# microsoft/fadtk

Measured on AMD Instinct MI355X. Metric: FAD scores/sec + cov-GEMM TFLOP/s (% MFMA peak), N=100k D=512, higher is better.
Workload: dtype f16 in, f16 MFMA with f32 accumulate over <= 8192-row runs, f64 across runs (moments); split-f16 MFMA iterations (f32 accumulate) + exact int8-MFMA products (int32 accumulate) + f64 correction (Frechet)

## Files before the change

fadtk_amd/csrc/frechet.hip:

```cpp
#include "frechet_internal.h"
#include "ns_mean.h"
#include "ns_fast.h"
#include "ns_fast_big.h"
#include "ns_fast_res.h"

#include <algorithm>
#include <atomic>
#include <cmath>
#include <type_traits>

namespace fad {

Pool& thread_pool(int device) {
    static thread_local PerThreadDevice<Pool> set;
    return set.get(device);
}
Workspace* free_slot(int device) {
    Pool& p = thread_pool(device);
    for (Workspace& w : p.slot)
        if (!w.busy) { w.pool = &p; return &w; }
    return nullptr;
}

SongKnobs SongKnobs::from_env() {
    SongKnobs k;
    auto off = [](const char* name) { const char* e = getenv(name); return e && e[0] == '0'; };
    if (const char* e = getenv("FAD_SONG_BIG")) k.big_min = atol(e);
    if (const char* e = getenv("FAD_SONG_RES")) k.res = (e[0] == '0') ? 0 : (e[0] == '1' ? 1 : 2);
    if (const char* e = getenv("FAD_SONG_FAST")) k.fast = (e[0] == '0') ? 0 : (e[0] == '2' ? 2 : 1);
    if (const char* e = getenv("FAD_FAST_TRACE")) k.trace = e[0] == '1';
    k.scaled = !off("FAD_SONG_SCALED");
    if (const char* e = getenv("FAD_SONG_L0_SCALE")) { const double v = atof(e); if (v > 0.0) k.l0_scale = v; }
    return k;
}


struct MixedResult {
    int status;
    int iters, decided_at, nonfinite, too_few0, too_few1;
    double tr_scaled, c, tr1, tr2, mean_term, res, est;
    int prepared;
    int pad;
};

__global__ __launch_bounds__(256) void ns32_finish(const double* __restrict__ stats, int d, int nb,
                                                   const NsState* __restrict__ st, Ns32State* __restrict__ s32,
                                                   MixedResult* __restrict__ out, int max_low) {
    __shared__ double red[4];
    __shared__ double red3[12];
    const int tid = threadIdx.x;
    const bool live = s32->ok != 0;
    double mr = 0.0, mc = 0.0, corr = 0.0, r2 = 0.0, tr = 0.0;
    if (live) {
        const double* rowabs = stats;
        const double* colabs = stats + (int64_t)nb * d;
        const double* scal = stats + 2 * (int64_t)nb * d;
// ... 211 lines not shown
    g.B[0] = Rv; g.C[0] = Pv; g.C[1] = Ev;
    fast_split(d, nsf::SP_V2, g, st, B);
    g.B[0] = Pv; g.A[1] = Ev; g.C[0] = nsf::SplitMat{nullptr, nullptr}; g.C[1] = nsf::SplitMat{nullptr, nullptr};
    fast_split(d, nsf::SP_V3, g, st, B);
}
static void fast_split(int d, int mode, const nsf::SplitArgs& g, hipStream_t st, unsigned B) {
    const unsigned t = (unsigned)(d / 32);
    switch (d) {
        case 128: fast_launch_split<1>(mode, t, B, g, st); break;
        case 256: fast_launch_split<2>(mode, t, B, g, st); break;
        case 384: fast_launch_split<3>(mode, t, B, g, st); break;
        case 512: fast_launch_split<4>(mode, t, B, g, st); break;
        case 768: fast_launch_split<6>(mode, t, B, g, st); break;
        default: fast_launch_split<8>(mode, t, B, g, st); break;
    }
}
template <int NJ> static void fast_big_attrs() {
    (void)hipFuncSetAttribute(reinterpret_cast<const void*>(&nsf::nsf_big<nsf::SP_T, NJ>), hipFuncAttributeMaxDynamicSharedMemorySize, (int)nsf::kBigLds);
    (void)hipFuncSetAttribute(reinterpret_cast<const void*>(&nsf::nsf_big<nsf::SP_U, NJ>), hipFuncAttributeMaxDynamicSharedMemorySize, (int)nsf::kBigLds);
    (void)hipFuncSetAttribute(reinterpret_cast<const void*>(&nsf::nsf_big<nsf::SP_FIRST, NJ>), hipFuncAttributeMaxDynamicSharedMemorySize, (int)nsf::kBigLds);
}
template <int NJ> static void fast_big_launch(int d, int mode, const nsf::SplitArgs& g, hipStream_t st, unsigned B) {
    const int tt = nsf::big_tiles(d, NJ);
    const unsigned one = (unsigned)nsf::big_grid((int)B, tt), two = (unsigned)nsf::big_grid((int)B, 2 * tt);
    if (mode == nsf::SP_FIRST) hipLaunchKernelGGL((nsf::nsf_big<nsf::SP_FIRST, NJ>), dim3(one), dim3(256), nsf::kBigLds, st, g);
    else if (mode == nsf::SP_T) hipLaunchKernelGGL((nsf::nsf_big<nsf::SP_T, NJ>), dim3(one), dim3(256), nsf::kBigLds, st, g);
    else hipLaunchKernelGGL((nsf::nsf_big<nsf::SP_U, NJ>), dim3(two + B), dim3(256), nsf::kBigLds, st, g);
}
static int fast_big_t_slots(int d, unsigned B) { return nsf::big_tiles(d, nsf::big_nj(d, 1, (int)B)); }
static int fast_split_big(int d, int mode, nsf::SplitArgs g, hipStream_t st, unsigned B, int device) {
    static std::atomic<unsigned> ready{0};
    if (device >= 0 && device < 32 && !(ready.load(std::memory_order_acquire) & (1u << device))) {
        fast_big_attrs<1>(); fast_big_attrs<2>();
        FAD_HIP_TRY(hipGetLastError());
        ready.fetch_or(1u << device, std::memory_order_release);
    }
    g.nprob = (int)B;
    if (nsf::big_nj(d, mode == nsf::SP_U ? 2 : 1, (int)B) == 1) fast_big_launch<1>(d, mode, g, st, B);
    else fast_big_launch<2>(d, mode, g, st, B);
    return FAD_OK;
}
static int fast_i8_big(int d, int mode, const nsf::I8Args& g, hipStream_t st, unsigned B, int device) {
    static std::atomic<unsigned> ready{0};
    if (device >= 0 && device < 32 && !(ready.load(std::memory_order_acquire) & (1u << device))) {
        FAD_HIP_TRY(hipFuncSetAttribute(reinterpret_cast<const void*>(&nsf::nsf_i8_big<nsf::I8_A>), hipFuncAttributeMaxDynamicSharedMemorySize, (int)nsf::kI8BigLds));
        FAD_HIP_TRY(hipFuncSetAttribute(reinterpret_cast<const void*>(&nsf::nsf_i8_big<nsf::I8_G>), hipFuncAttributeMaxDynamicSharedMemorySize, (int)nsf::kI8BigLds));
        FAD_HIP_TRY(hipFuncSetAttribute(reinterpret_cast<const void*>(&nsf::nsf_i8_big<nsf::I8_G, true>), hipFuncAttributeMaxDynamicSharedMemorySize, (int)nsf::kI8BigLds));
        ready.fetch_or(1u << device, std::memory_order_release);
    }
    const unsigned grid = (unsigned)nsf::big_grid((int)B, (d / 128) * (d / 64));
    if (mode == nsf::I8_A) hipLaunchKernelGGL((nsf::nsf_i8_big<nsf::I8_A>), dim3(grid), dim3(512), nsf::kI8BigLds, st, g, (int)B);
    else if (g.Rv.a) hipLaunchKernelGGL((nsf::nsf_i8_big<nsf::I8_G, true>), dim3(grid), dim3(512), nsf::kI8BigLds, st, g, (int)B);
    else hipLaunchKernelGGL((nsf::nsf_i8_big<nsf::I8_G>), dim3(grid), dim3(512), nsf::kI8BigLds, st, g, (int)B);
    return FAD_OK;
}
template <int NS8> static void fast_launch_i8(int mode, unsigned t, unsigned B, const nsf::I8Args& g, hipStream_t st) {
    if (mode == nsf::I8_A) hipLaunchKernelGGL((nsf::nsf_i8<NS8, nsf::I8_A>), dim3(t, t, B), dim3(512), 0, st, g);
    else hipLaunchKernelGGL((nsf::nsf_i8<NS8, nsf::I8_G>), dim3(t, t, B), dim3(512), 0, st, g);
}
static void fast_i8(int d, int mode, const nsf::I8Args& g, hipStream_t st, unsigned B = 1) {
    const unsigned t = (unsigned)(d / 32);
    switch (d) {
        case 128: case 256: fast_launch_i8<1>(mode, t, B, g, st); break;
        case 384: case 512: fast_launch_i8<2>(mode, t, B, g, st); break;
        case 768: fast_launch_i8<3>(mode, t, B, g, st); break;
        default: fast_launch_i8<4>(mode, t, B, g, st); break;
    }
}

static nsf::SplitArgs fast_split_args(Workspace& ws, const MixedBufs& m, const FastBufs& f, int d) {
    nsf::SplitArgs g;
    memset(&g, 0, sizeof(g));
    g.d = d; g.gen = ws.job.gen; g.hA = f.hdr; g.hB = f.hdr + 1; g.st = m.dstate; g.s32 = m.s32;
    if (wide_enabled(ws.pool)) { g.scaled = 1; g.lp_wide = 1; g.l0_scale = kWideL0Scale; g.l0_min = kWideL0Min; }
    return g;
}
static int fast_verify_enqueue(Workspace& ws) {
    const int d = ws.job.d;
    MixedBufs m = mixed_bufs(ws, d);
    FastBufs f = fast_bufs(ws, d);
    f.host_words[13] = 0;
    fast_verify_launch(d, 1, fast_split_args(ws, m, f, d), f.Y, f.Z, f.Rv, f.Pv, f.Ev, m.s32, f.host_vstats, f.host_words, 0, ws.job.stream);
    FAD_HIP_TRY(hipGetLastError());
    FAD_HIP_TRY(hipEventRecord(ws.done_ev, ws.job.stream));
    return FAD_OK;
}
static int fast_enqueue(Workspace& ws, int upto) {
    const int d = ws.job.d;
    hipStream_t stream = ws.job.stream;
    MixedBufs m = mixed_bufs(ws, d);
    FastBufs f = fast_bufs(ws, d);
    if (!f.host_words) return set_error(FAD_ERR_ALLOC, "pinned result area of the fast Frechet chain is missing");
    const int nslots = (d / 32) * (d / 32);
    const int max_low = max_low_of(ws);
    for (int& k = ws.job.k; k < upto; ++k) {
        nsf::SplitArgs g = fast_split_args(ws, m, f, d);
        if (k == 0) {
            nsf::I8Args a;
            memset(&a, 0, sizeof(a));
            a.Adig = f.digC[0]; a.Bdig = f.digC[1]; a.d = d; a.gen = ws.job.gen; a.hA = f.hdr; a.hB = f.hdr + 1; a.stats = m.tilestats;
            a.A64 = m.A; a.P = f.P; a.st = m.dstate;
            fast_i8(d, nsf::I8_A, a, stream);
            g.A[0] = f.P; g.B[0] = f.P; g.C[0] = f.Y[1]; g.C[1] = f.Z[1]; g.Cdig[0] = f.digY[1]; g.Cdig_t[0] = f.digYt[1];
            g.A64 = m.A; g.statsA = m.tilestats;
            fast_split(d, nsf::SP_FIRST, g, stream, 1);
            continue;
// ... 360 lines not shown
    char* hpin = static_cast<char*>(ws.fast_pairs_pin);
    double* h_vals = reinterpret_cast<double*>(hpin);
    double* h_stats = h_vals + nsf::kHostVals;
    int* h_words = reinterpret_cast<int*>(h_stats + (size_t)(nsf::kTileStats + 2) * nb * nb);
    auto at = [&](size_t off) { return blk + off; };
    auto mat = [&](size_t off) { nsf::SplitMat m; m.a = reinterpret_cast<uint4*>(at(off)); m.at = reinterpret_cast<uint4*>(at(off + 4 * dd)); return m; };
    const int gen = ++ws.fast_gen;
    if (ws.fast_gen > (1 << 30)) ws.fast_gen = 1;
    ws.multi.gen = gen;
    if (ws.fast_pairs.p != before) {
        FAD_HIP_TRY(hipMemset2DAsync(at(L.hdrA), L.stride, 0, sizeof(nsf::MatHdr), (size_t)B, st));
        FAD_HIP_TRY(hipMemset2DAsync(at(L.hdrB), L.stride, 0, sizeof(nsf::MatHdr), (size_t)B, st));
    }
    nsf::MatHdr* hA = reinterpret_cast<nsf::MatHdr*>(at(L.hdrA));
    nsf::MatHdr* hB = reinterpret_cast<nsf::MatHdr*>(at(L.hdrB));
    NsState* st0 = reinterpret_cast<NsState*>(at(L.st));
    Ns32State* s32_0 = reinterpret_cast<Ns32State*>(at(L.s32));
    double* partials = reinterpret_cast<double*>(at(L.partials));
    double* stats = reinterpret_cast<double*>(at(L.stats));
    double* A64 = reinterpret_cast<double*>(at(L.A64));
    const nsf::SplitMat P = mat(L.P), Y[2] = {mat(L.Y[0]), mat(L.Y[1])}, Z[2] = {mat(L.Z[0]), mat(L.Z[1])}, T = mat(L.T);
    uint4* digY[2] = {reinterpret_cast<uint4*>(at(L.digY[0])), reinterpret_cast<uint4*>(at(L.digY[1]))};
    uint4* digYt[2] = {reinterpret_cast<uint4*>(at(L.digYt[0])), reinterpret_cast<uint4*>(at(L.digYt[1]))};

    static_assert(2 * kMaxMultiPairs <= nsf::kPrepMaxSets, "PrepArgs holds two sets per pair of a batch");
    nsf::PrepArgs pa;
    memset(&pa, 0, sizeof(pa));
    for (int b = 0; b < B; ++b) {
        pa.accs[2 * b] = moments_packed(h1[b]); pa.accs[2 * b + 1] = moments_packed(h2[b]);
        pa.runs[2 * b] = moments_runsum(h1[b]); pa.runs[2 * b + 1] = moments_runsum(h2[b]);
    }
    pa.acc[0] = pa.accs[0]; pa.acc[1] = pa.accs[1];
    pa.d = d; pa.ddof = ddof; pa.gen = gen; pa.mean_dtype = mean_dtype;
    pa.mus = reinterpret_cast<double*>(at(L.mus)); pa.covs = reinterpret_cast<double*>(at(L.covs));
    pa.dig[0] = reinterpret_cast<uint4*>(at(L.digA)); pa.dig[1] = reinterpret_cast<uint4*>(at(L.digB));
    pa.st = st0; pa.hdr[0] = hA; pa.hdr[1] = hB;
    pa.batch = 2; pa.pstride = (int64_t)L.stride; pa.no_covs = 1;
    pa.per = ((dd / 2048) % 4 == 0) ? 4 : 2;
    hipLaunchKernelGGL(nsf::nsf_prepare, dim3((unsigned)(dd / 2048 / pa.per + 1), (unsigned)(2 * B)), dim3(512), 0, st, pa);

    auto split_args = [&]() {
        nsf::SplitArgs g;
        memset(&g, 0, sizeof(g));
        g.d = d; g.gen = gen; g.hA = hA; g.hB = hB; g.pstride = (int64_t)L.stride; g.astride = (int64_t)L.stride;
        g.st = st0; g.s32 = s32_0;
        if (wide) { g.scaled = 1; g.lp_wide = 1; g.l0_scale = kWideL0Scale; g.l0_min = kWideL0Min; }
        return g;
    };
    {
        nsf::I8Args a;
        memset(&a, 0, sizeof(a));
        a.Adig = reinterpret_cast<uint4*>(at(L.digA)); a.Bdig = reinterpret_cast<uint4*>(at(L.digB)); a.d = d; a.gen = gen; a.hA = hA; a.hB = hB;
        a.pstride = (int64_t)L.stride; a.astride = (int64_t)L.stride; a.stats = stats; a.A64 = A64; a.P = P; a.st = st0;
        if (big) FAD_TRY(fast_i8_big(d, nsf::I8_A, a, st, (unsigned)B, device));
        else fast_i8(d, nsf::I8_A, a, st, (unsigned)B);
        nsf::SplitArgs g = split_args();
        g.A[0] = P; g.B[0] = P; g.C[0] = Y[1]; g.C[1] = Z[1]; g.A64 = A64; g.statsA = stats;
        if (big) FAD_TRY(fast_split_big(d, nsf::SP_FIRST, g, st, (unsigned)B, device));
        else { g.Cdig[0] = digY[1]; g.Cdig_t[0] = digYt[1]; fast_split(d, nsf::SP_FIRST, g, st, (unsigned)B); }
    }
    int want = ws.pool ? ws.pool->lp_iters : 5;
    if (want < 2) want = 2;
    if (want > max_low) want = max_low;
    for (int k = 1; k < want; ++k) {
        const int cur = k & 1;
        nsf::SplitArgs g = split_args();
        g.A[0] = Z[cur]; g.B[0] = Y[cur]; g.C[0] = T; g.alpha = -0.5f; g.beta_eye = 1.5f; g.gamma = 1.0f;
        g.partials = partials; g.skip = &s32_0->done; g.k = k;
        if (big) FAD_TRY(fast_split_big(d, nsf::SP_T, g, st, (unsigned)B, device));
        else fast_split(d, nsf::SP_T, g, st, (unsigned)B);
        g = split_args();
        g.A[0] = Y[cur]; g.B[0] = T; g.C[0] = Y[cur ^ 1]; g.A[1] = T; g.B[1] = Z[cur]; g.C[1] = Z[cur ^ 1];
        if (!big) { g.Cdig[0] = digY[cur ^ 1]; g.Cdig_t[0] = digYt[cur ^ 1]; }
        g.skip = &s32_0->upd_skip[k & 1];
        g.k = k; g.max_low = max_low; g.nslots = big ? fast_big_t_slots(d, (unsigned)B) : nb * nb; g.chk_partials = partials; g.thr_pred = pred_threshold(ws.pool, d);
        if (big) FAD_TRY(fast_split_big(d, nsf::SP_U, g, st, (unsigned)B, device));
        else fast_split(d, nsf::SP_U, g, st, (unsigned)B);
    }
    if (big) {
        nsf::DigArgs dg;
        memset(&dg, 0, sizeof(dg));
        dg.d = d; dg.gen = gen; dg.hA = hA; dg.hB = hB; dg.pstride = (int64_t)L.stride; dg.astride = (int64_t)L.stride; dg.s32 = s32_0;
        dg.Y[0] = Y[0]; dg.Y[1] = Y[1]; dg.dig[0] = digY[0]; dg.dig[1] = digY[1]; dg.dig_t[0] = digYt[0]; dg.dig_t[1] = digYt[1];
        hipLaunchKernelGGL(nsf::nsf_digitize, dim3((unsigned)((dd / 16 + 255) / 256), 2, (unsigned)B), dim3(256), 0, st, dg);
    }
    {
        nsf::I8Args a;
        memset(&a, 0, sizeof(a));
        a.Adig = digY[0]; a.Bdig = digYt[0]; a.Adig_alt = digY[1]; a.Bdig_alt = digYt[1]; a.sel = &s32_0->final_iter;
        a.d = d; a.gen = gen; a.hA = hA; a.hB = hB; a.pstride = (int64_t)L.stride; a.astride = (int64_t)L.stride; a.hstride = (int64_t)hs;
        a.skip = &s32_0->skip_corr; a.stats = h_stats; a.st = st0; a.A64in = A64;
        a.Y[0] = Y[0]; a.Y[1] = Y[1]; a.Z[0] = Z[0]; a.Z[1] = Z[1]; a.s32 = s32_0; a.host_words = h_words; a.host_vals = h_vals;
        if (wide) { a.Rv = mat(L.Rv); a.scaled = 1; }
        for (int b = 0; b < B; ++b) { int* w = reinterpret_cast<int*>(reinterpret_cast<char*>(h_words) + (size_t)b * hs); w[12] = 0; w[13] = 0; }
        if (big) FAD_TRY(fast_i8_big(d, nsf::I8_G, a, st, (unsigned)B, device));
        else fast_i8(d, nsf::I8_G, a, st, (unsigned)B);
    }
    FAD_HIP_TRY(hipGetLastError());
    if (!ws.done_ev) FAD_HIP_TRY(hipEventCreateWithFlags(&ws.done_ev, hipEventDisableTiming));
    if (wide && ws.pool && ws.pool->lp_verify) return pairs_verify_enqueue(ws, d, B, st);
    FAD_HIP_TRY(hipEventRecord(ws.done_ev, st));
    return FAD_OK;
}

static int mixed_begin(const NsProblem& pb, int device, hipStream_t stream, Workspace& ws) {
    const int d = pb.d;
    const int64_t dd = (int64_t)d * d;
    FAD_TRY(ws.mats.reserve((size_t)(6 * dd) * sizeof(double)));
    FAD_TRY(ws.mats32.reserve((size_t)(5 * dd) * sizeof(float)));
    const size_t hbytes = ws.job.fast ? fast_pinned_bytes(d) : sizeof(NsState) + sizeof(MixedResult);
    if (!ws.pinned || ws.pinned_cap < hbytes) {
        if (ws.pinned) (void)hipHostFree(ws.pinned);
        ws.pinned = nullptr; ws.pinned_cap = 0;
        FAD_HIP_TRY(hipHostMalloc(&ws.pinned, hbytes + 4096, hipHostMallocDefault));
        ws.pinned_cap = hbytes + 4096;
    }
    MixedBufs m = mixed_bufs(ws, d);
    m.hres->status = -1;
    ws.job.d = d; ws.job.device = device; ws.job.stream = stream; ws.job.k = 0;
    if (ws.job.fast) {
        ws.job.mu1 = pb.mu1; ws.job.mu2 = pb.mu2; ws.job.mean_dtype = pb.mean_dtype;
        int want = ws.pool ? ws.pool->lp_iters : 5;
        if (want < 2) want = 2;
        if (want > max_low_of(ws)) want = max_low_of(ws);
        if (ws.pool && ws.pool->lp_hopeless) want = 1;
        return fast_enqueue(ws, want);
    }
    NsProductExt ext;
    memset(&ext, 0, sizeof(ext));
    ext.stats = m.tilestats; ext.mu1 = pb.mu1; ext.mu2 = pb.mu2; ext.mean_dtype = pb.mean_dtype; ext.st = m.dstate;
    FAD_TRY(gemm_f64_product_stats_launch(d, pb.cov1, pb.cov2, m.A, &m.dstate->done, ext, stream));
    enqueue_ns_prepare(m.tilestats, d, (int)m.nb, pb.mu1, 0, pb.mu2, 0, pb.mean_dtype, m.dstate, 1, m.s32, 1, stream);
    int want = ws.pool ? ws.pool->lp_iters : 5;
    if (want < 2) want = 2;
    if (want > kMaxLow) want = kMaxLow;
    return mixed_enqueue(ws, want);
}

static int mixed_finish(Workspace& ws, MixedResult* res) {
    MixedBufs m = mixed_bufs(ws, ws.job.d);
    const int max_low = max_low_of(ws);
    bool asked = false;
    for (;;) {
        FAD_HIP_TRY(hipEventSynchronize(ws.done_ev));
        if (ws.job.fast) FAD_TRY(fast_decide(ws));
        if (m.hres->status == 5) {
            if (asked) { m.hres->status = 2; break; }
            asked = true;
// ... 383 lines not shown
```

fadtk_amd/csrc/ns_fast_big.h:

```cpp
#pragma once
#include "ns_fast.h"
#include "big_slots.h"

namespace fad {
namespace nsf {

#ifndef FAD_BIG_STAGES
#define FAD_BIG_STAGES 3
#endif
constexpr int kBigStages = FAD_BIG_STAGES;
constexpr int kBigStage = 1024;
constexpr size_t kBigLds = (size_t)kBigStages * kBigStage * 16 + 256;

template <int MODE, int NJ = 2>
__global__ __launch_bounds__(256, (FAD_BIG_STAGES <= 3) ? 3 : ((FAD_BIG_STAGES <= 4) ? 2 : 1)) void nsf_big(SplitArgs g) {
    static_assert(MODE == SP_T || MODE == SP_U || MODE == SP_FIRST, "SP_FIRST: iteration 0 (scale from nsf_i8<A>'s statistics, Y1, Z1)");
    extern __shared__ __attribute__((aligned(16))) uint4 ring[];
    double* red = reinterpret_cast<double*>(ring + kBigStages * kBigStage);
    const int d = g.d, tid = threadIdx.x, lane = tid & 63;
    constexpr int ZP = (MODE == SP_U) ? 2 : 1;
    const int t = d >> 7, tx_n = (NJ == 2) ? t : 2 * t, tt = t * tx_n;
    const int L = blockIdx.x;
    const int nprod = big_grid(g.nprob, tt * ZP);
    if constexpr (MODE == SP_U) {
// ... 176 lines not shown
                for (int reg = 0; reg < 16; ++reg) {
                    const int q = (reg & 3) + 8 * (reg >> 2);
                    const float y0 = (float)(A64[(int64_t)q * d] * inv_c);
                    const float y2 = (float)((double)(acc0[i][j][reg] + acc1[i][j][reg] * kLoInv) * (inv_cn * inv_cn));
                    fin[(q + 4 * kg) * 33 + r] = m1 * y0 - m3 * y2;
                    z1[reg] = ((by == bx && q + 4 * kg == r) ? m1 : 0.f) - m3 * y0;
                }
                __builtin_amdgcn_wave_barrier();
#pragma unroll
                for (int pass = 0; pass < 4; ++pass) store_tile_planes(fin, Cm, by, bx, d, pass * 64 + lane);
                __builtin_amdgcn_wave_barrier();
#pragma unroll
                for (int reg = 0; reg < 16; ++reg) fin[((reg & 3) + 8 * (reg >> 2) + 4 * kg) * 33 + r] = z1[reg];
                __builtin_amdgcn_wave_barrier();
                const SplitMat Zm1 = adv(g.C[1], po);
#pragma unroll
                for (int pass = 0; pass < 4; ++pass) store_tile_planes(fin, Zm1, by, bx, d, pass * 64 + lane);
                __builtin_amdgcn_wave_barrier();
                continue;
            }
            float ssf = 0.f;
#pragma unroll
            for (int reg = 0; reg < 16; ++reg) {
                const int q = (reg & 3) + 8 * (reg >> 2) + 4 * kg;
                const bool dg = (by == bx) && (q == r);
                const float v = alpha * (acc0[i][j][reg] + acc1[i][j][reg] * kLoInv) + (dg ? beta : 0.f);
                if constexpr (MODE == SP_T) { const float e = v - (dg ? gamma : 0.f); ssf = __builtin_fmaf(e, e, ssf); }
                fin[q * 33 + r] = v;
            }
            ss += (double)ssf;
            __builtin_amdgcn_wave_barrier();
#pragma unroll
            for (int pass = 0; pass < 4; ++pass) store_tile_planes(fin, Cm, by, bx, d, pass * 64 + lane);
            if (with_digits) {
#pragma unroll 2
                for (int pass = 0; pass < 8; ++pass) store_tile_digits(fin, dig, dig_t, by, bx, d, pass * 64 + lane);
            }
            __builtin_amdgcn_wave_barrier();
        }
    if constexpr (MODE == SP_T) {
        double s1[1] = {ss};
        wg8_sum<1, 4>(s1, red);
        if (tid == 0) adv(g.partials, po)[tile] = s1[0];
    }
}

constexpr int kI8BigStage = 36 * 64;
#ifndef FAD_I8_BIG_STAGES
#define FAD_I8_BIG_STAGES 2
#endif
constexpr int kI8BigStages = FAD_I8_BIG_STAGES;
constexpr size_t kI8BigLds = (size_t)kI8BigStages * kI8BigStage * 16 + 256;

template <int MODE, bool WITHR = false>
__global__ __launch_bounds__(512) void nsf_i8_big(I8Args g, int nprob) {
    extern __shared__ __attribute__((aligned(16))) uint4 ring[];
    double* red = reinterpret_cast<double*>(ring + kI8BigStages * kI8BigStage);
    constexpr int kUmin = (MODE == I8_A) ? kUminA : kUminG;
    constexpr int kGroups = 2 * (kDigits - 1) - kUmin + 1;
    const int d = g.d, tid = threadIdx.x, lane = tid & 63;
    const int tr_ = d >> 7, tc_ = d >> 6, tt = tr_ * tc_;
    const BigSlot slot = big_slot(blockIdx.x, nprob, tt);
    if (!slot.live) return;
    const int song = slot.song, tile = slot.item;
    const int TY = tile / tc_, TX = tile - TY * tc_;
    const int64_t po = (int64_t)song * g.pstride, ho = (int64_t)song * g.hstride;
    const MatHdr* hB = adv(g.hB, po);
    const MatHdr* hA = adv(g.hA, (int64_t)song * g.astride);
    NsState* const st_p = adv(g.st, po);
    const bool bad = hdr_bad(hA, hB, g.gen);
    const bool skipped = bad || (g.skip && *adv(g.skip, po) != 0);
    if constexpr (MODE == I8_G) {
        if (tile == 0 && tid == 0) {
            const NsState* st = st_p; const Ns32State* s = adv(g.s32, po);
            int* hw = adv(g.host_words, ho); double* hv = adv(g.host_vals, ho);
            hw[0] = bad ? 1 : 0; hw[1] = st->done; hw[2] = st->nonfinite; hw[3] = st->too_few[0]; hw[4] = st->too_few[1];
            hw[5] = s->ok; hw[6] = s->failed; hw[7] = s->final_iter; hw[8] = s->decided_at; hw[9] = s->strict; hw[10] = s->finished;
            hw[11] = skipped ? 1 : 0;
            hv[0] = st->c; hv[1] = st->tr1; hv[2] = st->tr2; hv[3] = st->mean_term;
#pragma unroll
            for (int q = 0; q < 16; ++q) hv[4 + q] = s->res[q];
            hw[14] = (g.scaled && st->mu[0] != 1.0) ? 1 : 0;
            hw[12] = g.gen;
        }
    }
    if (skipped) return;
    const int wave = __builtin_amdgcn_readfirstlane(tid >> 6);
    const int wr = wave >> 1, wc = wave & 1;
    const bool alt = (MODE == I8_G) && g.sel && (*adv(g.sel, po) & 1);
    const uint4* Ad = (MODE == I8_A) ? adv(g.Adig, (int64_t)song * g.astride) : adv(alt ? g.Adig_alt : g.Adig, po);
    const uint4* Bd = adv(alt ? g.Bdig_alt : g.Bdig, po);
#ifdef FAD_I8_ABL_G_NOLOOP
    const int nks = (MODE == I8_G) ? 0 : (d >> 5);
#else
    const int nks = d >> 5;
#endif

    const uint32_t voff = (uint32_t)lane * 16u;
    const uint32_t ring_lds = (uint32_t)(size_t)(__attribute__((address_space(3))) void*)ring;
    auto issue = [&](int ks) {
#pragma unroll
        for (int i = 0; i < 5; ++i) {
            const int q = wave + 8 * i;
            if (q < 36) {
                const bool bs = q >= 24;
                const int blk = bs ? (q - 24) / 6 : q / 6, p = bs ? (q - 24) % 6 : q % 6;
                const uint64_t sb = (uint64_t)((bs ? Bd : Ad) + dg_idx((bs ? 2 * TX : 4 * TY) + blk, ks, p, 0, d));
                const uint32_t lo = __builtin_amdgcn_readfirstlane((uint32_t)sb);
                const uint32_t hi = __builtin_amdgcn_readfirstlane((uint32_t)(sb >> 32));
                const uint64_t ub = ((uint64_t)hi << 32) | lo;
                const uint32_t m0v = __builtin_amdgcn_readfirstlane(ring_lds + (uint32_t)(((ks % kI8BigStages) * kI8BigStage + q * 64) * 16));
                asm volatile("s_mov_b32 m0, %2\n\ts_nop 0\n\tglobal_load_lds_dwordx4 %0, %1" ::"v"(voff), "s"(ub), "s"(m0v) : "memory", "m0");
            }
        }
    };
    i32x16 acc[kGroups];
#pragma unroll
    for (int u = 0; u < kGroups; ++u)
#pragma unroll
        for (int q = 0; q < 16; ++q) acc[u][q] = 0;
    static_assert(kI8BigStages >= 2 && kI8BigStages <= 4, "the counted waits below cover two younger stages at most");
    for (int ks = 0; ks < kI8BigStages - 1 && ks < nks; ++ks) issue(ks);
    const bool five = wave < 4;
    for (int ks = 0; ks < nks; ++ks) {
        const int ahead = (nks - 1 - ks < kI8BigStages - 2) ? (nks - 1 - ks) : (kI8BigStages - 2);
        if (ahead == 2) { if (five) asm volatile("s_waitcnt vmcnt(10)" ::: "memory"); else asm volatile("s_waitcnt vmcnt(8)" ::: "memory"); }
        else if (ahead == 1) { if (five) asm volatile("s_waitcnt vmcnt(5)" ::: "memory"); else asm volatile("s_waitcnt vmcnt(4)" ::: "memory"); }
        else asm volatile("s_waitcnt vmcnt(0)" ::: "memory");
        __builtin_amdgcn_s_barrier();
#ifndef FAD_I8_ABL_NODMA
        if (ks + kI8BigStages - 1 < nks) issue(ks + kI8BigStages - 1);
#endif
        const i32x4* st = reinterpret_cast<const i32x4*>(ring + (ks % kI8BigStages) * kI8BigStage) + lane;
        i32x4 a[kDigits], b[kDigits];
#pragma unroll
        for (int p = 0; p < kDigits; ++p) { a[p] = st[(wr * 6 + p) * 64]; b[p] = st[(24 + wc * 6 + p) * 64]; }
#ifdef FAD_I8_ABL_NOMMA
#pragma unroll
        for (int p = 0; p < kDigits; ++p) { acc[0][p] += a[p][0] ^ b[p][1]; acc[1][p] += a[p][2] ^ b[p][3]; }
#else
#pragma unroll
        for (int p = kDigits - 1; p >= 0; --p)
#pragma unroll
            for (int q = kDigits - 1; q >= 0; --q)
                if (p + q >= kUmin) acc[p + q - kUmin] = __builtin_amdgcn_mfma_i32_32x32x32_i8(a[p], b[q], acc[p + q - kUmin], 0, 0, 0);
#endif
    }
    __syncthreads();
    double gp[16];
#pragma unroll
    for (int q = 0; q < 16; ++q) gp[q] = 0.0;
#pragma unroll
    for (int u = 0; u < kGroups; ++u) {
        const double wgt = __builtin_ldexp(1.0, 7 * (u + kUmin) - 80);
#pragma unroll
        for (int q = 0; q < 16; ++q) gp[q] = __builtin_fma((double)acc[u][q], wgt, gp[q]);
    }
    float* fin = reinterpret_cast<float*>(ring) + wave * (32 * 33 + 32);
    const int kg = lane >> 5, n = lane & 31;
    const int by = 4 * TY + wr, bx = 2 * TX + wc, nb = d >> 5;
    const int row0 = 32 * by, col0 = 32 * bx;
    double* const stats = adv(g.stats, (MODE == I8_A) ? po : ho);
    double* scal = stats + (size_t)kTileStats * (by * nb + bx);
    double v3[3] = {0.0, 0.0, 0.0};
    if constexpr (MODE == I8_A) {
        const double inv = hdr_inv_s12(hA, hB);
        double* A64 = adv(g.A64, po) + (int64_t)(row0 + 4 * kg) * d + col0 + n;
#pragma unroll
        for (int reg = 0; reg < 16; ++reg) {
            const int q = (reg & 3) + 8 * (reg >> 2);
            A64[(int64_t)q * d] = gp[reg] * inv;
            fin[(q + 4 * kg) * 33 + n] = (float)gp[reg];
            v3[0] += gp[reg] * gp[reg];
            if (by == bx && q + 4 * kg == n) v3[1] += gp[reg];
        }
        __builtin_amdgcn_wave_barrier();
        const SplitMat Pm = adv(g.P, po);
#pragma unroll
        for (int pass = 0; pass < 4; ++pass) store_tile_planes(fin, Pm, by, bx, d, pass * 64 + lane);
    } else {
        const SplitMat Zm = adv(g.Z[alt ? 1 : 0], po);
        const SplitMat Ym = adv(g.Y[alt ? 1 : 0], po);
        const double inv_c = 1.0 / st_p->c;
        const double* A64 = adv(g.A64in, po) + (int64_t)(row0 + 4 * kg) * d + col0 + n;
        typedef _Float16 f16x4 __attribute__((ext_vector_type(4)));
        f16x4 zh[4], zl[4];
#pragma unroll
        for (int j = 0; j < 4; ++j) {
            int half;
            const size_t zi = fa_elem(col0 + n, row0 + 8 * j + 4 * kg, 0, d, half);
            zh[j] = *reinterpret_cast<const f16x4*>(reinterpret_cast<const _Float16*>(Zm.a + zi) + half);
            zl[j] = *reinterpret_cast<const f16x4*>(reinterpret_cast<const _Float16*>(Zm.a + zi + 64) + half);
        }
#pragma unroll
        for (int reg = 0; reg < 16; ++reg) {
            const int q = (reg & 3) + 8 * (reg >> 2), gr = row0 + q + 4 * kg, gc = col0 + n;
            const double R = A64[(int64_t)q * d] * inv_c - gp[reg];
            if constexpr (WITHR) gp[reg] = R;
            const double z = (double)used16(zh[reg >> 2][reg & 3], zl[reg >> 2][reg & 3]);
            v3[0] += z * R; v3[1] += R * R;
            if (by == bx && gr == gc) {
                int hy;
                const size_t yi = fa_elem(gr, gr, 0, d, hy);
                v3[2] += (double)used16(reinterpret_cast<const _Float16*>(Ym.a + yi)[hy], reinterpret_cast<const _Float16*>(Ym.a + yi + 64)[hy]);
            }
            fin[(q + 4 * kg) * 33 + n] = fabsf((float)z);
        }
        __builtin_amdgcn_wave_barrier();
    }
    double m = 0.0;
    if constexpr (MODE == I8_A) {
        if (lane < 32) { for (int c = 0; c < 32; ++c) m += fabsf(fin[lane * 33 + c]); }
        else { for (int q = 0; q < 32; ++q) m += fabsf(fin[q * 33 + lane - 32]); }
    } else {
        if (lane < 32) { for (int q = 0; q < 32; ++q) m += fin[q * 33 + lane]; }
        else { for (int c = 0; c < 32; ++c) m += fin[(lane - 32) * 33 + c]; }
    }
    double mrow = (lane < 32) ? m : 0.0, mcol = (lane >= 32) ? m : 0.0;
#pragma unroll
    for (int off = 32; off > 0; off >>= 1) {
        mrow = fmax(mrow, __shfl_xor(mrow, off)); mcol = fmax(mcol, __shfl_xor(mcol, off));
#pragma unroll
        for (int q = 0; q < 3; ++q) v3[q] += __shfl_xor(v3[q], off);
    }
    if (lane == 0) {
        if constexpr (MODE == I8_A) {
            scal[0] = v3[0]; scal[1] = v3[1]; scal[2] = mrow; scal[3] = mcol;
        } else {
            scal[0] = v3[0]; scal[1] = v3[1]; scal[2] = v3[2]; scal[3] = 0.0;
            double* zmax = stats + (size_t)kTileStats * nb * nb + 2 * (size_t)(by * nb + bx);
            zmax[0] = mrow; zmax[1] = mcol;
        }
    }
    if constexpr (MODE == I8_G && WITHR) {
        if (g.Rv.a) {
            __builtin_amdgcn_wave_barrier();
#pragma unroll
            for (int reg = 0; reg < 16; ++reg) fin[((reg & 3) + 8 * (reg >> 2) + 4 * kg) * 33 + n] = (float)(gp[reg] * (double)kVerScale);
            __builtin_amdgcn_wave_barrier();
            const SplitMat Rm = adv(g.Rv, po);
#pragma unroll
            for (int pass = 0; pass < 4; ++pass) store_tile_planes(fin, Rm, by, bx, d, pass * 64 + lane);
        }
    }
    (void)red;
}

}
}
```

Baseline: 12910.

## Add 64x64-tile int8 pair kernel with two-stage ring for big Frechet path

Adds a new int8 MFMA kernel for the big-matrix path. It uses 256 threads (4 waves covering a 64x64 output tile) instead of 512 threads on 128x64 tiles, with a two-stage LDS ring and launch bounds asking for 3 blocks per CU. The goal is more blocks in flight and a smaller LDS footprint, so more of the CUs stay busy at moderate d. In exchange each block reuses loaded digits less and the pipelining is shallower, since it waits on vmcnt(0) every k-step. The shared epilogue and per-problem setup are moved into helpers so both kernels can use them.

```diff
diff --git a/fadtk_amd/csrc/frechet.hip b/fadtk_amd/csrc/frechet.hip
--- a/fadtk_amd/csrc/frechet.hip
+++ b/fadtk_amd/csrc/frechet.hip
@@ -2,6 +2,7 @@
 #include "ns_mean.h"
 #include "ns_fast.h"
 #include "ns_fast_big.h"
+#include "ns_i8_pairs.h"
 #include "ns_fast_res.h"
 
 #include <algorithm>
@@ -319,6 +320,20 @@
     if (mode == nsf::I8_A) hipLaunchKernelGGL((nsf::nsf_i8_big<nsf::I8_A>), dim3(grid), dim3(512), nsf::kI8BigLds, st, g, (int)B);
     else if (g.Rv.a) hipLaunchKernelGGL((nsf::nsf_i8_big<nsf::I8_G, true>), dim3(grid), dim3(512), nsf::kI8BigLds, st, g, (int)B);
     else hipLaunchKernelGGL((nsf::nsf_i8_big<nsf::I8_G>), dim3(grid), dim3(512), nsf::kI8BigLds, st, g, (int)B);
+    return FAD_OK;
+}
+static int fast_i8_pairs(int d, int mode, const nsf::I8Args& g, hipStream_t st, unsigned B, int device) {
+    static std::atomic<unsigned> ready{0};
+    if (device >= 0 && device < 32 && !(ready.load(std::memory_order_acquire) & (1u << device))) {
+        FAD_HIP_TRY(hipFuncSetAttribute(reinterpret_cast<const void*>(&nsf::nsf_i8_pairs<nsf::I8_A>), hipFuncAttributeMaxDynamicSharedMemorySize, (int)nsf::kI8PairsLds));
+        FAD_HIP_TRY(hipFuncSetAttribute(reinterpret_cast<const void*>(&nsf::nsf_i8_pairs<nsf::I8_G>), hipFuncAttributeMaxDynamicSharedMemorySize, (int)nsf::kI8PairsLds));
+        FAD_HIP_TRY(hipFuncSetAttribute(reinterpret_cast<const void*>(&nsf::nsf_i8_pairs<nsf::I8_G, true>), hipFuncAttributeMaxDynamicSharedMemorySize, (int)nsf::kI8PairsLds));
+        ready.fetch_or(1u << device, std::memory_order_release);
+    }
+    const unsigned grid = (unsigned)nsf::big_grid((int)B, nsf::i8_pairs_tiles(d));
+    if (mode == nsf::I8_A) hipLaunchKernelGGL((nsf::nsf_i8_pairs<nsf::I8_A>), dim3(grid), dim3(256), nsf::kI8PairsLds, st, g, (int)B);
+    else if (g.Rv.a) hipLaunchKernelGGL((nsf::nsf_i8_pairs<nsf::I8_G, true>), dim3(grid), dim3(256), nsf::kI8PairsLds, st, g, (int)B);
+    else hipLaunchKernelGGL((nsf::nsf_i8_pairs<nsf::I8_G>), dim3(grid), dim3(256), nsf::kI8PairsLds, st, g, (int)B);
     return FAD_OK;
 }
 template <int NS8> static void fast_launch_i8(int mode, unsigned t, unsigned B, const nsf::I8Args& g, hipStream_t st) {
@@ -785,7 +800,7 @@
         memset(&a, 0, sizeof(a));
         a.Adig = reinterpret_cast<uint4*>(at(L.digA)); a.Bdig = reinterpret_cast<uint4*>(at(L.digB)); a.d = d; a.gen = gen; a.hA = hA; a.hB = hB;
         a.pstride = (int64_t)L.stride; a.astride = (int64_t)L.stride; a.stats = stats; a.A64 = A64; a.P = P; a.st = st0;
-        if (big) FAD_TRY(fast_i8_big(d, nsf::I8_A, a, st, (unsigned)B, device));
+        if (big) FAD_TRY(fast_i8_pairs(d, nsf::I8_A, a, st, (unsigned)B, device));
         else fast_i8(d, nsf::I8_A, a, st, (unsigned)B);
         nsf::SplitArgs g = split_args();
         g.A[0] = P; g.B[0] = P; g.C[0] = Y[1]; g.C[1] = Z[1]; g.A64 = A64; g.statsA = stats;
@@ -826,7 +841,7 @@
         a.Y[0] = Y[0]; a.Y[1] = Y[1]; a.Z[0] = Z[0]; a.Z[1] = Z[1]; a.s32 = s32_0; a.host_words = h_words; a.host_vals = h_vals;
         if (wide) { a.Rv = mat(L.Rv); a.scaled = 1; }
         for (int b = 0; b < B; ++b) { int* w = reinterpret_cast<int*>(reinterpret_cast<char*>(h_words) + (size_t)b * hs); w[12] = 0; w[13] = 0; }
-        if (big) FAD_TRY(fast_i8_big(d, nsf::I8_G, a, st, (unsigned)B, device));
+        if (big) FAD_TRY(fast_i8_pairs(d, nsf::I8_G, a, st, (unsigned)B, device));
         else fast_i8(d, nsf::I8_G, a, st, (unsigned)B);
     }
     FAD_HIP_TRY(hipGetLastError());
diff --git a/fadtk_amd/csrc/ns_fast_big.h b/fadtk_amd/csrc/ns_fast_big.h
--- a/fadtk_amd/csrc/ns_fast_big.h
+++ b/fadtk_amd/csrc/ns_fast_big.h
@@ -252,6 +252,151 @@
 constexpr int kI8BigStages = FAD_I8_BIG_STAGES;
 constexpr size_t kI8BigLds = (size_t)kI8BigStages * kI8BigStage * 16 + 256;
 
+struct I8Prob {
+    int64_t po, ho;
+    const MatHdr* hA; const MatHdr* hB;
+    NsState* st;
+    bool skipped, alt;
+};
+template <int MODE>
+__device__ __forceinline__ I8Prob i8_problem(const I8Args& g, int song, bool first) {
+    I8Prob pb;
+    const int64_t po = (int64_t)song * g.pstride, ho = (int64_t)song * g.hstride;
+    pb.po = po; pb.ho = ho;
+    pb.hB = adv(g.hB, po);
+    pb.hA = adv(g.hA, (int64_t)song * g.astride);
+    pb.st = adv(g.st, po);
+    const bool bad = hdr_bad(pb.hA, pb.hB, g.gen);
+    const bool skipped = bad || (g.skip && *adv(g.skip, po) != 0);
+    pb.skipped = skipped;
+    if constexpr (MODE == I8_G) {
+        if (first) {
+            const NsState* st = pb.st; const Ns32State* s = adv(g.s32, po);
+            int* hw = adv(g.host_words, ho); double* hv = adv(g.host_vals, ho);
+            hw[0] = bad ? 1 : 0; hw[1] = st->done; hw[2] = st->nonfinite; hw[3] = st->too_few[0]; hw[4] = st->too_few[1];
+            hw[5] = s->ok; hw[6] = s->failed; hw[7] = s->final_iter; hw[8] = s->decided_at; hw[9] = s->strict; hw[10] = s->finished;
+            hw[11] = skipped ? 1 : 0;
+            hv[0] = st->c; hv[1] = st->tr1; hv[2] = st->tr2; hv[3] = st->mean_term;
+#pragma unroll
+            for (int q = 0; q < 16; ++q) hv[4 + q] = s->res[q];
+            hw[14] = (g.scaled && st->mu[0] != 1.0) ? 1 : 0;
+            hw[12] = g.gen;
+        }
+    }
+    pb.alt = false;
+    if constexpr (MODE == I8_G) { if (!skipped) pb.alt = g.sel && (*adv(g.sel, po) & 1); }
+    return pb;
+}
+
+template <int MODE, bool WITHR, int NG>
+__device__ __forceinline__ void i8_block_epilogue(const I8Args& g, const I8Prob& pb, const i32x16 (&acc)[NG], uint4* ring, int by, int bx, int wave) {
+    constexpr int kUmin = (MODE == I8_A) ? kUminA : kUminG;
+    constexpr int kGroups = NG;
+    static_assert(NG == 2 * (kDigits - 1) - kUmin + 1, "one accumulator per digit-pair weight");
+    const int d = g.d, lane = threadIdx.x & 63;
+    const int64_t po = pb.po, ho = pb.ho;
+    const MatHdr* hA = pb.hA; const MatHdr* hB = pb.hB;
+    const NsState* st_p = pb.st;
+    const bool alt = pb.alt;
+    __syncthreads();
+    double gp[16];
+#pragma unroll
+    for (int q = 0; q < 16; ++q) gp[q] = 0.0;
+#pragma unroll
+    for (int u = 0; u < kGroups; ++u) {
+        const double wgt = __builtin_ldexp(1.0, 7 * (u + kUmin) - 80);
+#pragma unroll
+        for (int q = 0; q < 16; ++q) gp[q] = __builtin_fma((double)acc[u][q], wgt, gp[q]);
+    }
+    float* fin = reinterpret_cast<float*>(ring) + wave * (32 * 33 + 32);
+    const int kg = lane >> 5, n = lane & 31;
+    const int nb = d >> 5;
+    const int row0 = 32 * by, col0 = 32 * bx;
+    double* const stats = adv(g.stats, (MODE == I8_A) ? po : ho);
+    double* scal = stats + (size_t)kTileStats * (by * nb + bx);
+    double v3[3] = {0.0, 0.0, 0.0};
+    if constexpr (MODE == I8_A) {
+        const double inv = hdr_inv_s12(hA, hB);
+        double* A64 = adv(g.A64, po) + (int64_t)(row0 + 4 * kg) * d + col0 + n;
+#pragma unroll
+        for (int reg = 0; reg < 16; ++reg) {
+            const int q = (reg & 3) + 8 * (reg >> 2);
+            A64[(int64_t)q * d] = gp[reg] * inv;
+            fin[(q + 4 * kg) * 33 + n] = (float)gp[reg];
+            v3[0] += gp[reg] * gp[reg];
+            if (by == bx && q + 4 * kg == n) v3[1] += gp[reg];
+        }
+        __builtin_amdgcn_wave_barrier();
+        const SplitMat Pm = adv(g.P, po);
+#pragma unroll
+        for (int pass = 0; pass < 4; ++pass) store_tile_planes(fin, Pm, by, bx, d, pass * 64 + lane);
+    } else {
+        const SplitMat Zm = adv(g.Z[alt ? 1 : 0], po);
+        const SplitMat Ym = adv(g.Y[alt ? 1 : 0], po);
+        const double inv_c = 1.0 / st_p->c;
+        const double* A64 = adv(g.A64in, po) + (int64_t)(row0 + 4 * kg) * d + col0 + n;
+        typedef _Float16 f16x4 __attribute__((ext_vector_type(4)));
+        f16x4 zh[4], zl[4];
+#pragma unroll
+        for (int j = 0; j < 4; ++j) {
+            int half;
+            const size_t zi = fa_elem(col0 + n, row0 + 8 * j + 4 * kg, 0, d, half);
+            zh[j] = *reinterpret_cast<const f16x4*>(reinterpret_cast<const _Float16*>(Zm.a + zi) + half);
+            zl[j] = *reinterpret_cast<const f16x4*>(reinterpret_cast<const _Float16*>(Zm.a + zi + 64) + half);
+        }
+#pragma unroll
+        for (int reg = 0; reg < 16; ++reg) {
+            const int q = (reg & 3) + 8 * (reg >> 2), gr = row0 + q + 4 * kg, gc = col0 + n;
+            const double R = A64[(int64_t)q * d] * inv_c - gp[reg];
+            if constexpr (WITHR) gp[reg] = R;
+            const double z = (double)used16(zh[reg >> 2][reg & 3], zl[reg >> 2][reg & 3]);
+            v3[0] += z * R; v3[1] += R * R;
+            if (by == bx && gr == gc) {
+                int hy;
+                const size_t yi = fa_elem(gr, gr, 0, d, hy);
+                v3[2] += (double)used16(reinterpret_cast<const _Float16*>(Ym.a + yi)[hy], reinterpret_cast<const _Float16*>(Ym.a + yi + 64)[hy]);
+            }
+            fin[(q + 4 * kg) * 33 + n] = fabsf((float)z);
+        }
+        __builtin_amdgcn_wave_barrier();
+    }
+    double m = 0.0;
+    if constexpr (MODE == I8_A) {
+        if (lane < 32) { for (int c = 0; c < 32; ++c) m += fabsf(fin[lane * 33 + c]); }
+        else { for (int q = 0; q < 32; ++q) m += fabsf(fin[q * 33 + lane - 32]); }
+    } else {
+        if (lane < 32) { for (int q = 0; q < 32; ++q) m += fin[q * 33 + lane]; }
+        else { for (int c = 0; c < 32; ++c) m += fin[(lane - 32) * 33 + c]; }
+    }
+    double mrow = (lane < 32) ? m : 0.0, mcol = (lane >= 32) ? m : 0.0;
+#pragma unroll
+    for (int off = 32; off > 0; off >>= 1) {
+        mrow = fmax(mrow, __shfl_xor(mrow, off)); mcol = fmax(mcol, __shfl_xor(mcol, off));
+#pragma unroll
+        for (int q = 0; q < 3; ++q) v3[q] += __shfl_xor(v3[q], off);
+    }
+    if (lane == 0) {
+        if constexpr (MODE == I8_A) {
+            scal[0] = v3[0]; scal[1] = v3[1]; scal[2] = mrow; scal[3] = mcol;
+        } else {
+            scal[0] = v3[0]; scal[1] = v3[1]; scal[2] = v3[2]; scal[3] = 0.0;
+            double* zmax = stats + (size_t)kTileStats * nb * nb + 2 * (size_t)(by * nb + bx);
+            zmax[0] = mrow; zmax[1] = mcol;
+        }
+    }
+    if constexpr (MODE == I8_G && WITHR) {
+        if (g.Rv.a) {
+            __builtin_amdgcn_wave_barrier();
+#pragma unroll
+            for (int reg = 0; reg < 16; ++reg) fin[((reg & 3) + 8 * (reg >> 2) + 4 * kg) * 33 + n] = (float)(gp[reg] * (double)kVerScale);
+            __builtin_amdgcn_wave_barrier();
+            const SplitMat Rm = adv(g.Rv, po);
+#pragma unroll
+            for (int pass = 0; pass < 4; ++pass) store_tile_planes(fin, Rm, by, bx, d, pass * 64 + lane);
+        }
+    }
+}
+
 template <int MODE, bool WITHR = false>
 __global__ __launch_bounds__(512) void nsf_i8_big(I8Args g, int nprob) {
     extern __shared__ __attribute__((aligned(16))) uint4 ring[];
@@ -264,30 +409,12 @@
     if (!slot.live) return;
     const int song = slot.song, tile = slot.item;
     const int TY = tile / tc_, TX = tile - TY * tc_;
-    const int64_t po = (int64_t)song * g.pstride, ho = (int64_t)song * g.hstride;
-    const MatHdr* hB = adv(g.hB, po);
-    const MatHdr* hA = adv(g.hA, (int64_t)song * g.astride);
-    NsState* const st_p = adv(g.st, po);
-    const bool bad = hdr_bad(hA, hB, g.gen);
-    const bool skipped = bad || (g.skip && *adv(g.skip, po) != 0);
-    if constexpr (MODE == I8_G) {
-        if (tile == 0 && tid == 0) {
-            const NsState* st = st_p; const Ns32State* s = adv(g.s32, po);
-            int* hw = adv(g.host_words, ho); double* hv = adv(g.host_vals, ho);
-            hw[0] = bad ? 1 : 0; hw[1] = st->done; hw[2] = st->nonfinite; hw[3] = st->too_few[0]; hw[4] = st->too_few[1];
-            hw[5] = s->ok; hw[6] = s->failed; hw[7] = s->final_iter; hw[8] = s->decided_at; hw[9] = s->strict; hw[10] = s->finished;
-            hw[11] = skipped ? 1 : 0;
-            hv[0] = st->c; hv[1] = st->tr1; hv[2] = st->tr2; hv[3] = st->mean_term;
-#pragma unroll
-            for (int q = 0; q < 16; ++q) hv[4 + q] = s->res[q];
-            hw[14] = (g.scaled && st->mu[0] != 1.0) ? 1 : 0;
-            hw[12] = g.gen;
-        }
-    }
-    if (skipped) return;
+    const I8Prob pb = i8_problem<MODE>(g, song, tile == 0 && tid == 0);
+    if (pb.skipped) return;
+    const int64_t po = pb.po;
     const int wave = __builtin_amdgcn_readfirstlane(tid >> 6);
     const int wr = wave >> 1, wc = wave & 1;
-    const bool alt = (MODE == I8_G) && g.sel && (*adv(g.sel, po) & 1);
+    const bool alt = pb.alt;
     const uint4* Ad = (MODE == I8_A) ? adv(g.Adig, (int64_t)song * g.astride) : adv(alt ? g.Adig_alt : g.Adig, po);
     const uint4* Bd = adv(alt ? g.Bdig_alt : g.Bdig, po);
 #ifdef FAD_I8_ABL_G_NOLOOP
@@ -346,103 +473,7 @@
                 if (p + q >= kUmin) acc[p + q - kUmin] = __builtin_amdgcn_mfma_i32_32x32x32_i8(a[p], b[q], acc[p + q - kUmin], 0, 0, 0);
 #endif
     }
-    __syncthreads();
-    double gp[16];
-#pragma unroll
-    for (int q = 0; q < 16; ++q) gp[q] = 0.0;
-#pragma unroll
-    for (int u = 0; u < kGroups; ++u) {
-        const double wgt = __builtin_ldexp(1.0, 7 * (u + kUmin) - 80);
-#pragma unroll
-        for (int q = 0; q < 16; ++q) gp[q] = __builtin_fma((double)acc[u][q], wgt, gp[q]);
-    }
-    float* fin = reinterpret_cast<float*>(ring) + wave * (32 * 33 + 32);
-    const int kg = lane >> 5, n = lane & 31;
-    const int by = 4 * TY + wr, bx = 2 * TX + wc, nb = d >> 5;
-    const int row0 = 32 * by, col0 = 32 * bx;
-    double* const stats = adv(g.stats, (MODE == I8_A) ? po : ho);
-    double* scal = stats + (size_t)kTileStats * (by * nb + bx);
-    double v3[3] = {0.0, 0.0, 0.0};
-    if constexpr (MODE == I8_A) {
-        const double inv = hdr_inv_s12(hA, hB);
-        double* A64 = adv(g.A64, po) + (int64_t)(row0 + 4 * kg) * d + col0 + n;
-#pragma unroll
-        for (int reg = 0; reg < 16; ++reg) {
-            const int q = (reg & 3) + 8 * (reg >> 2);
-            A64[(int64_t)q * d] = gp[reg] * inv;
-            fin[(q + 4 * kg) * 33 + n] = (float)gp[reg];
-            v3[0] += gp[reg] * gp[reg];
-            if (by == bx && q + 4 * kg == n) v3[1] += gp[reg];
-        }
-        __builtin_amdgcn_wave_barrier();
-        const SplitMat Pm = adv(g.P, po);
-#pragma unroll
-        for (int pass = 0; pass < 4; ++pass) store_tile_planes(fin, Pm, by, bx, d, pass * 64 + lane);
-    } else {
-        const SplitMat Zm = adv(g.Z[alt ? 1 : 0], po);
-        const SplitMat Ym = adv(g.Y[alt ? 1 : 0], po);
-        const double inv_c = 1.0 / st_p->c;
-        const double* A64 = adv(g.A64in, po) + (int64_t)(row0 + 4 * kg) * d + col0 + n;
-        typedef _Float16 f16x4 __attribute__((ext_vector_type(4)));
-        f16x4 zh[4], zl[4];
-#pragma unroll
-        for (int j = 0; j < 4; ++j) {
-            int half;
-            const size_t zi = fa_elem(col0 + n, row0 + 8 * j + 4 * kg, 0, d, half);
-            zh[j] = *reinterpret_cast<const f16x4*>(reinterpret_cast<const _Float16*>(Zm.a + zi) + half);
-            zl[j] = *reinterpret_cast<const f16x4*>(reinterpret_cast<const _Float16*>(Zm.a + zi + 64) + half);
-        }
-#pragma unroll
-        for (int reg = 0; reg < 16; ++reg) {
-            const int q = (reg & 3) + 8 * (reg >> 2), gr = row0 + q + 4 * kg, gc = col0 + n;
-            const double R = A64[(int64_t)q * d] * inv_c - gp[reg];
-            if constexpr (WITHR) gp[reg] = R;
-            const double z = (double)used16(zh[reg >> 2][reg & 3], zl[reg >> 2][reg & 3]);
-            v3[0] += z * R; v3[1] += R * R;
-            if (by == bx && gr == gc) {
-                int hy;
-                const size_t yi = fa_elem(gr, gr, 0, d, hy);
-                v3[2] += (double)used16(reinterpret_cast<const _Float16*>(Ym.a + yi)[hy], reinterpret_cast<const _Float16*>(Ym.a + yi + 64)[hy]);
-            }
-            fin[(q + 4 * kg) * 33 + n] = fabsf((float)z);
-        }
-        __builtin_amdgcn_wave_barrier();
-    }
-    double m = 0.0;
-    if constexpr (MODE == I8_A) {
-        if (lane < 32) { for (int c = 0; c < 32; ++c) m += fabsf(fin[lane * 33 + c]); }
-        else { for (int q = 0; q < 32; ++q) m += fabsf(fin[q * 33 + lane - 32]); }
-    } else {
-        if (lane < 32) { for (int q = 0; q < 32; ++q) m += fin[q * 33 + lane]; }
-        else { for (int c = 0; c < 32; ++c) m += fin[(lane - 32) * 33 + c]; }
-    }
-    double mrow = (lane < 32) ? m : 0.0, mcol = (lane >= 32) ? m : 0.0;
-#pragma unroll
-    for (int off = 32; off > 0; off >>= 1) {
-        mrow = fmax(mrow, __shfl_xor(mrow, off)); mcol = fmax(mcol, __shfl_xor(mcol, off));
-#pragma unroll
-        for (int q = 0; q < 3; ++q) v3[q] += __shfl_xor(v3[q], off);
-    }
-    if (lane == 0) {
-        if constexpr (MODE == I8_A) {
-            scal[0] = v3[0]; scal[1] = v3[1]; scal[2] = mrow; scal[3] = mcol;
-        } else {
-            scal[0] = v3[0]; scal[1] = v3[1]; scal[2] = v3[2]; scal[3] = 0.0;
-            double* zmax = stats + (size_t)kTileStats * nb * nb + 2 * (size_t)(by * nb + bx);
-            zmax[0] = mrow; zmax[1] = mcol;
-        }
-    }
-    if constexpr (MODE == I8_G && WITHR) {
-        if (g.Rv.a) {
-            __builtin_amdgcn_wave_barrier();
-#pragma unroll
-            for (int reg = 0; reg < 16; ++reg) fin[((reg & 3) + 8 * (reg >> 2) + 4 * kg) * 33 + n] = (float)(gp[reg] * (double)kVerScale);
-            __builtin_amdgcn_wave_barrier();
-            const SplitMat Rm = adv(g.Rv, po);
-#pragma unroll
-            for (int pass = 0; pass < 4; ++pass) store_tile_planes(fin, Rm, by, bx, d, pass * 64 + lane);
-        }
-    }
+    i8_block_epilogue<MODE, WITHR>(g, pb, acc, ring, 4 * TY + wr, 2 * TX + wc, wave);
     (void)red;
 }
 
diff --git a/fadtk_amd/csrc/ns_i8_pairs.h b/fadtk_amd/csrc/ns_i8_pairs.h
--- /dev/null
+++ b/fadtk_amd/csrc/ns_i8_pairs.h
@@ -0,0 +1,72 @@
+#pragma once
+#include "ns_fast_big.h"
+
+namespace fad {
+namespace nsf {
+
+constexpr int kI8PairsStage = 24 * 64;
+constexpr int kI8PairsStages = 2;
+constexpr size_t kI8PairsLds = (size_t)kI8PairsStages * kI8PairsStage * 16 + 256;
+constexpr int i8_pairs_tiles(int d) { return (d >> 6) * (d >> 6); }
+static_assert(4 * (32 * 33 + 32) * sizeof(float) <= (size_t)kI8PairsStages * kI8PairsStage * 16, "the epilogue's four [32][33] areas live in the ring");
+
+template <int MODE, bool WITHR = false>
+__global__ __launch_bounds__(256, 3) void nsf_i8_pairs(I8Args g, int nprob) {
+    extern __shared__ __attribute__((aligned(16))) uint4 ring[];
+    constexpr int kUmin = (MODE == I8_A) ? kUminA : kUminG;
+    constexpr int kGroups = 2 * (kDigits - 1) - kUmin + 1;
+    const int d = g.d, tid = threadIdx.x, lane = tid & 63;
+    const int tc_ = d >> 6;
+    const BigSlot slot = big_slot(blockIdx.x, nprob, tc_ * tc_);
+    if (!slot.live) return;
+    const int song = slot.song, tile = slot.item;
+    const int TY = tile / tc_, TX = tile - TY * tc_;
+    const I8Prob pb = i8_problem<MODE>(g, song, tile == 0 && tid == 0);
+    if (pb.skipped) return;
+    const int wave = __builtin_amdgcn_readfirstlane(tid >> 6);
+    const int wr = wave >> 1, wc = wave & 1;
+    const uint4* Ad = (MODE == I8_A) ? adv(g.Adig, (int64_t)song * g.astride) : adv(pb.alt ? g.Adig_alt : g.Adig, pb.po);
+    const uint4* Bd = adv(pb.alt ? g.Bdig_alt : g.Bdig, pb.po);
+    const int nks = d >> 5;
+
+    const uint32_t voff = (uint32_t)lane * 16u;
+    const uint32_t ring_lds = (uint32_t)(size_t)(__attribute__((address_space(3))) void*)ring;
+    auto issue = [&](int ks) {
+#pragma unroll
+        for (int i = 0; i < 6; ++i) {
+            const int q = wave + 4 * i;
+            const bool bs = q >= 12;
+            const int blk = bs ? (q - 12) / 6 : q / 6, p = bs ? (q - 12) % 6 : q % 6;
+            const uint64_t sb = (uint64_t)((bs ? Bd : Ad) + dg_idx(2 * (bs ? TX : TY) + blk, ks, p, 0, d));
+            const uint32_t lo = __builtin_amdgcn_readfirstlane((uint32_t)sb);
+            const uint32_t hi = __builtin_amdgcn_readfirstlane((uint32_t)(sb >> 32));
+            const uint64_t ub = ((uint64_t)hi << 32) | lo;
+            const uint32_t m0v = __builtin_amdgcn_readfirstlane(ring_lds + (uint32_t)(((ks % kI8PairsStages) * kI8PairsStage + q * 64) * 16));
+            asm volatile("s_mov_b32 m0, %2\n\ts_nop 0\n\tglobal_load_lds_dwordx4 %0, %1" ::"v"(voff), "s"(ub), "s"(m0v) : "memory", "m0");
+        }
+    };
+    i32x16 acc[kGroups];
+#pragma unroll
+    for (int u = 0; u < kGroups; ++u)
+#pragma unroll
+        for (int q = 0; q < 16; ++q) acc[u][q] = 0;
+    issue(0);
+    for (int ks = 0; ks < nks; ++ks) {
+        asm volatile("s_waitcnt vmcnt(0)" ::: "memory");
+        __builtin_amdgcn_s_barrier();
+        if (ks + 1 < nks) issue(ks + 1);
+        const i32x4* st = reinterpret_cast<const i32x4*>(ring + (ks % kI8PairsStages) * kI8PairsStage) + lane;
+        i32x4 a[kDigits], b[kDigits];
+#pragma unroll
+        for (int p = 0; p < kDigits; ++p) { a[p] = st[(wr * 6 + p) * 64]; b[p] = st[(12 + wc * 6 + p) * 64]; }
+#pragma unroll
+        for (int p = kDigits - 1; p >= 0; --p)
+#pragma unroll
+            for (int q = kDigits - 1; q >= 0; --q)
+                if (p + q >= kUmin) acc[p + q - kUmin] = __builtin_amdgcn_mfma_i32_32x32x32_i8(a[p], b[q], acc[p + q - kUmin], 0, 0, 0);
+    }
+    i8_block_epilogue<MODE, WITHR>(g, pb, acc, ring, 2 * TY + wr, 2 * TX + wc, wave);
+}
+
+}
+}
```

Result: slower. 12660 (-1.9%).
